# felipescoelho/w-ofdm-optimization

Hardware: AMD Instinct MI355X
Metric: OFDM symbols/sec (whole node) + BER vs reference, N=256 16-QAM (higher is better)
Workload: dtype f32

## Files before the change

include/wofdm.h:

```cpp
#ifndef WOFDM_H
#define WOFDM_H

#include <stdint.h>

#ifdef __cplusplus
extern "C" {
#endif

#define WOFDM_ABI_VERSION 1

#define WOFDM_OK            0
#define WOFDM_E_INVALID    -1
#define WOFDM_E_UNSUPPORTED -2
#define WOFDM_E_HIP        -3
#define WOFDM_E_NOMEM      -4

#define WOFDM_MAX_TAPS     21
#define WOFDM_MAX_SYMS     16

typedef struct wofdm_cfg {
    int32_t  n_fft;
    int32_t  bits_per_sc;
    int32_t  syms_per_frame;
    int32_t  cp, cs;
// ... 45 lines not shown

int wofdm_plan_dump_frame(wofdm_plan *plan, uint32_t cell, uint64_t frame,
                          const uint8_t *labels, const float *unit_noise,
                          uint64_t *counts, wofdm_dump *out);

int wofdm_plan_set_allocation(wofdm_plan *plan, const uint8_t *active);

int wofdm_plan_set_tx_mask(wofdm_plan *plan, const float *mask);

int wofdm_plan_status(wofdm_plan *plan);

int wofdm_plan_info(wofdm_plan *plan, int32_t info[5]);

int wofdm_plan_kernel_id(wofdm_plan *plan, int32_t id[2]);

int wofdm_plan_kernel_geo(wofdm_plan *plan, int32_t *id);
int wofdm_cfg_geo_id(const wofdm_cfg *cfg);

#define WOFDM_OPT_FIR_VALU       0
#define WOFDM_OPT_MAX_SPW        1
#define WOFDM_OPT_TXMASK_DIRECT  2
#define WOFDM_OPT_DFT_VALU       3
#define WOFDM_OPT_GENERIC_GEOMETRY 4
int wofdm_plan_set_option(wofdm_plan *plan, int32_t option, int32_t value);

int wofdm_run(const wofdm_cfg *cfg, int device, const float *w_tx, const float *w_rx,
              const float *h, const float *snr_db, uint64_t *counts);
int wofdm_run_injected(const wofdm_cfg *cfg, int device, const float *w_tx, const float *w_rx,
                       const float *h, const float *snr_db, const uint8_t *labels,
                       const float *unit_noise, uint64_t *counts);

int wofdm_interference(const wofdm_cfg *cfg, int device, const float *w_tx, const float *w_rx,
                       const float *h, float *power);

int wofdm_interference_masked(const wofdm_cfg *cfg, int device, const float *w_tx, const float *w_rx,
                              const float *h, const uint8_t *active ,
                              const float *tx_mask ,
                              float *power  ,
                              float *wanted );

int wofdm_tx_psd(const wofdm_cfg *cfg, int device, const float *w_tx, const float *X, int no_symbols,
                 int overlap, float *psd);

typedef struct wofdm_psd_job {
    int32_t block;
    int32_t cp, cs;
    int32_t overlap;
// ... 353 lines not shown
```

w-ofdm-optimization_amd/_lib.py:

```python
import ctypes as C
import os
import subprocess

import numpy as np

_HERE = os.path.dirname(os.path.abspath(__file__))
LIB_PATH = os.environ.get("WOFDM_LIB", os.path.join(_HERE, "libwofdm_hip.so"))
_LIB = None

WOFDM_OK = 0
ERRORS = {-1: "WOFDM_E_INVALID", -2: "WOFDM_E_UNSUPPORTED", -3: "WOFDM_E_HIP", -4: "WOFDM_E_NOMEM"}
MAX_TAPS = 21
OPTIONS = {"fir_valu": 0, "max_spw": 1, "txmask_direct": 2, "dft_valu": 3, "generic_geometry": 4}
MAX_SYMS = 16
TX_PAPR_CHUNK_BYTES = 256 << 20
TX_PAPR_MAX_PERIODS = 1 << 20
RX_PROFILE_CHUNK_BYTES = 256 << 20
SYNC_MAX_POINTS = 64
DOPPLER_MAX_TRACKS = 16
DOPPLER_MAX_KNOTS = 64
PA_LINEAR, PA_RAPP, PA_CLIP = 0, 1, 2
PA_MAX_POINTS = 16
PN_MAX_POINTS = 16
LINK_MAX_POINTS = 16
SOFT_MAX_SCALES = 16
CODE_MAX = 4
CODE_MAX_STEPS = 4608
CODE_LONG_MAX_STEPS = 1048576
LDPC_MAX_BITS = 16384

EXPORTS = (
    "wofdm_version", "wofdm_device_count", "wofdm_last_error", "wofdm_noise_len",
    "wofdm_plan_create", "wofdm_plan_destroy", "wofdm_plan_launch", "wofdm_plan_launch_timed",
    "wofdm_plan_launch_injected", "wofdm_plan_dump_frame", "wofdm_plan_info", "wofdm_run",
    "wofdm_run_injected", "wofdm_philox_kat", "wofdm_plan_set_allocation",
    "wofdm_plan_set_tx_mask", "wofdm_plan_status", "wofdm_plan_kernel_id", "wofdm_plan_set_option",
    "wofdm_interference", "wofdm_tx_psd", "wofdm_tx_psd_batch", "wofdm_tx_psd_batch_masked",
    "wofdm_interference_masked", "wofdm_tx_papr", "wofdm_tx_papr_kernel_ms",
    "wofdm_rx_profile", "wofdm_rx_profile_kernel_ms", "wofdm_plan_kernel_geo", "wofdm_cfg_geo_id",
    "wofdm_rx_profile_aci", "wofdm_rx_profile_sync", "wofdm_rx_profile_doppler",
    "wofdm_rx_profile_pa", "wofdm_tx_psd_batch_pa", "wofdm_rx_profile_pn",
    "wofdm_rx_profile_link", "wofdm_rx_profile_soft", "wofdm_rx_profile_tracking",
    "wofdm_rx_profile_coded", "wofdm_code_steps", "wofdm_viterbi_decode",
    "wofdm_viterbi_decode_long", "wofdm_rx_profile_coded_frame",
    "wofdm_ldpc_lift", "wofdm_ldpc_decode", "wofdm_rx_profile_ldpc",
)


class WofdmError(RuntimeError):
    def __init__(self, code, message):
        super().__init__("%s (%d): %s" % (ERRORS.get(code, "WOFDM_E_?"), code, message))
        self.code = code


class Cfg(C.Structure):
    _fields_ = [(n, C.c_int32) for n in (
        "n_fft", "bits_per_sc", "syms_per_frame", "cp", "cs", "tail_tx", "tail_rx", "prefix_rm",
        "circ_shift", "n_taps", "n_channels", "n_snr", "n_window_pairs",
        "noise_before_truncate")] + [
        ("frames_per_cell", C.c_uint64), ("frame_offset", C.c_uint64), ("seed", C.c_uint64)]

    @property
    def sym_len(self):
        return self.n_fft + self.cp + self.cs

    @property
    def stride(self):
        return self.sym_len - self.tail_tx
# ... 70 lines not shown
        import torch
    except ImportError:
        pass
    if not os.path.exists(LIB_PATH):
        raise ImportError(
            "%s not found: build it with `make -C %s` (hipcc, gfx950). The w-OFDM hot path has "
            "no CPU fallback." % (LIB_PATH, os.path.join(_HERE, "csrc")))
    L = C.CDLL(LIB_PATH)
    vp, u64 = C.c_void_p, C.c_uint64
    L.wofdm_version.restype = C.c_int
    L.wofdm_device_count.restype = C.c_int
    L.wofdm_last_error.restype = C.c_char_p
    L.wofdm_noise_len.argtypes = [C.POINTER(Cfg)]
    L.wofdm_plan_create.argtypes = [C.POINTER(vp), C.POINTER(Cfg), C.c_int, vp, vp, vp, vp]
    L.wofdm_plan_destroy.argtypes = [vp]
    L.wofdm_plan_launch.argtypes = [vp, u64, u64, vp, vp]
    L.wofdm_plan_launch_timed.argtypes = [vp, u64, u64, vp, vp, C.POINTER(C.c_float)]
    L.wofdm_plan_launch_injected.argtypes = [vp, u64, vp, vp, vp, vp]
    L.wofdm_plan_dump_frame.argtypes = [vp, C.c_uint32, u64, vp, vp, vp, C.POINTER(Dump)]
    L.wofdm_plan_info.argtypes = [vp, vp]
    L.wofdm_plan_kernel_id.argtypes = [vp, vp]
    L.wofdm_plan_kernel_geo.argtypes = [vp, C.POINTER(C.c_int32)]
    L.wofdm_cfg_geo_id.argtypes = [C.POINTER(Cfg)]
    L.wofdm_plan_set_allocation.argtypes = [vp, vp]
    L.wofdm_plan_set_tx_mask.argtypes = [vp, vp]
    L.wofdm_plan_status.argtypes = [vp]
    L.wofdm_plan_set_option.argtypes = [vp, C.c_int32, C.c_int32]
    L.wofdm_run.argtypes = [C.POINTER(Cfg), C.c_int, vp, vp, vp, vp, vp]
    L.wofdm_run_injected.argtypes = [C.POINTER(Cfg), C.c_int, vp, vp, vp, vp, vp, vp, vp]
    L.wofdm_philox_kat.argtypes = [C.c_int, vp, vp, vp]
    L.wofdm_interference.argtypes = [C.POINTER(Cfg), C.c_int, vp, vp, vp, vp]
    L.wofdm_interference_masked.argtypes = [C.POINTER(Cfg), C.c_int, vp, vp, vp, vp, vp, vp, vp]
    L.wofdm_tx_psd.argtypes = [C.POINTER(Cfg), C.c_int, vp, vp, C.c_int, C.c_int, vp]
    i32 = C.c_int32
    L.wofdm_tx_psd_batch.argtypes = [i32, C.c_int, i32, vp, vp, i32, i32, vp, vp]
    L.wofdm_tx_psd_batch_masked.argtypes = [i32, C.c_int, i32, vp, vp, i32, vp, vp, vp, i32, i32, vp, vp]
    L.wofdm_tx_papr.argtypes = [C.POINTER(Cfg), C.c_int, vp, vp, vp, C.c_float, C.c_float, i32, vp, vp, vp]
    L.wofdm_tx_papr_kernel_ms.argtypes = [C.POINTER(C.c_float)]
    L.wofdm_rx_profile.argtypes = [C.POINTER(Cfg), C.c_int, vp, vp, vp, vp, vp, vp, vp, vp]
    L.wofdm_rx_profile_aci.argtypes = [C.POINTER(Cfg), C.c_int, vp, vp, vp, vp, vp, vp, vp, vp, i32, C.c_float, vp, vp]
    L.wofdm_rx_profile_kernel_ms.argtypes = [C.POINTER(C.c_float)]
    L.wofdm_rx_profile_sync.argtypes = [C.POINTER(Cfg), C.c_int, vp, vp, vp, vp, vp, vp, i32, C.POINTER(SyncPoint), vp, vp, vp, vp]
    L.wofdm_rx_profile_doppler.argtypes = [C.POINTER(Cfg), C.c_int, vp, vp, vp, i32, i32, i32, vp, vp, vp, vp, vp, vp, vp]
    L.wofdm_rx_profile_pa.argtypes = [C.POINTER(Cfg), C.c_int, vp, vp, vp, vp, vp, vp, i32, C.POINTER(PaPoint), vp, vp, vp, vp, vp, vp]
    L.wofdm_rx_profile_pn.argtypes = [C.POINTER(Cfg), C.c_int, vp, vp, vp, vp, vp, vp, i32, C.POINTER(PnPoint), vp, vp, vp, vp]
    L.wofdm_rx_profile_link.argtypes = [C.POINTER(Cfg), C.c_int, vp, vp, vp, vp, vp, vp, vp, i32, i32, i32, vp, vp, vp, i32,
# ... 45 lines not shown
```

w-ofdm-optimization_amd/csrc/wofdm_abi.hip:

```cpp
#include "../../include/wofdm.h"
#include "wofdm_kernel.h"
#include "wofdm_link.h"
#include "philox.h"

#include <algorithm>
#include <cmath>
#include <complex>
#include <cstdarg>
#include <cstdio>
#include <cstdlib>
#include <cstring>
#include <mutex>
#include <utility>
#include <vector>

namespace {

thread_local char g_err[512] = "";
thread_local float g_papr_ms = 0.f;
thread_local float g_rxprof_ms = 0.f;

int fail(int code, const char *fmt, ...)
{
    va_list ap;
// ... 63 lines not shown
    geom g{};
    uint32_t n_cells = 0;
    float *d_wtx = nullptr, *d_wrx = nullptr, *d_nlin = nullptr;
    float2 *d_h = nullptr;
    int *d_geo = nullptr;
    float2 *d_nscr = nullptr;
    uint64_t nscr_elems = 0;
    wofdm_kparams base{};
    wofdm_kernel_fn fn[4] = {nullptr, nullptr, nullptr, nullptr};
    int var = WOFDM_VAR_PLAIN;
    bool has_alloc = false, has_mask = false;
    bool force_direct_mask = false;
    bool fir_valu = false;
    bool dft_valu = false;
    int max_spw = 0;
    bool generic_geo = false;
    int geo = 0;
    uint32_t *d_amask = nullptr;
    float2 *d_tmask = nullptr;
    float2 *d_tspec = nullptr;
    float *d_tspec4 = nullptr;
    unsigned *d_status = nullptr;
    unsigned long long *d_work = nullptr;
    uint32_t split_alpha_256 = WOFDM_SPLIT_ALPHA_256, split_chunk = WOFDM_SPLIT_CHUNK;
    bool split_forced = false;
    uint4 *d_fira = nullptr;
    float firm_sx = 1.f, firm_sh = 1.f;
    uint4 *d_dftc = nullptr;
    float *d_rxs = nullptr;
#ifdef WOFDM_AUDIT
    uint32_t *audit = nullptr;
    uint32_t audit_items = 0;
#endif
    int occ = 1, cus = 1, layout = 1;
    hipEvent_t ev0 = nullptr, ev1 = nullptr;
};

namespace {

size_t wofdm_amask_words(int N)
{
    const size_t NQ = (size_t)N / 4;
    return N == 256 ? 2 * NQ + 256 : NQ + (NQ > 256 ? NQ : 256);
}

int geo_id_of(const geom &g)
// ... 109 lines not shown
    fft_pow2(a, -1);
    fft_pow2(b, -1);
    for (size_t i = 0; i < Mb; ++i) a[i] *= b[i];
    fft_pow2(a, +1);
    std::vector<cplx> g((size_t)L);
    for (int n = 0; n < L; ++n) g[(size_t)n] = a[(size_t)n] * c[(size_t)n] / ((double)Mb * (double)L);
    return g;
}

void mask_fastconv_spectrum(const float *mask, int L, int MF, float2 *spec)
{
    const int P = (L + 1) / 2, G = 3 * P - 2;
    const std::vector<cplx> g = idft_any(mask, L);
    std::vector<cplx> gt((size_t)MF, cplx(0.0, 0.0));
    for (int t = 0; t < G && t < MF; ++t) gt[(size_t)t] = g[(size_t)(((t - (P - 1)) % L + L) % L)];
    fft_pow2(gt, -1);
    for (int f = 0; f < MF; ++f)
        spec[f] = make_float2((float)(gt[(size_t)f].real() / MF), (float)(gt[(size_t)f].imag() / MF));
}

std::mutex g_gate_mu;
hipEvent_t g_gate_last[64] = {};

int launch(wofdm_plan *pl, int mode, wofdm_kparams &kp, uint64_t total_items, int force_grid,
           hipStream_t stream)
{
    wofdm_kernel_fn fn = pl->fn[mode];
    if (!fn) return fail(WOFDM_E_UNSUPPORTED, "no kernel for n_fft=%d", pl->g.N);
    if (total_items == 0) return WOFDM_OK;
    uint64_t grid = (uint64_t)pl->cus * (uint64_t)pl->occ;
#ifdef WOFDM_DEV_OCC
    grid = (uint64_t)pl->cus * (uint64_t)(WOFDM_DEV_OCC);
#endif
    if (grid > total_items) grid = total_items;
    if (force_grid > 0) grid = (uint64_t)force_grid;
    const size_t row = wofdm_noise_scratch_len(pl->g.N, pl->layout);
    if (row && grid * row > pl->nscr_elems) {
        HIP_TRY(hipDeviceSynchronize());
        if (pl->d_nscr) (void)hipFree(pl->d_nscr);
        pl->d_nscr = nullptr; pl->nscr_elems = 0;
        HIP_TRY(hipMalloc(&pl->d_nscr, grid * row * sizeof(float2)));
        pl->nscr_elems = grid * row;
    }
    kp.noise_scratch = pl->d_nscr;
    kp.status = pl->d_status;
    kp.dftc = pl->d_dftc;
    kp.rx_scale = pl->d_rxs;
    const bool dynamic = (mode == WOFDM_MODE_GEN || mode == WOFDM_MODE_INJECT) && wofdm_layout_dynamic(pl->layout, pl->g.N)
                         && (pl->split_forced || (pl->occ >= 2 && total_items / grid >= WOFDM_SPLIT_MIN_ITEMS));
    const wofdm_split sp = wofdm_work_split(total_items, grid, dynamic, pl->split_alpha_256, pl->split_chunk);
    kp.head_q = sp.head_q; kp.head_r = sp.head_r; kp.tail0 = sp.tail0; kp.total = total_items;
    kp.chunk = sp.chunk;
    kp.work = pl->d_work;
    kp.lds_bytes = pl->base.lds_bytes;
    float2 *tm = pl->var == WOFDM_VAR_TXFFT ? (pl->layout == 15 ? reinterpret_cast<float2 *>(pl->d_tspec4) : pl->d_tspec) : pl->d_tmask;
    kp.tx_scale = pl->base.tx_scale;
    kp.dump_unscale_tx = pl->base.dump_unscale_tx;
    kp.dump_unscale_rx = pl->base.dump_unscale_rx;
#ifdef WOFDM_AUDIT
    kp.audit = pl->audit; kp.audit_items = pl->audit_items;
#endif
#ifdef WOFDM_DELAY
    {
        const char *dp = std::getenv("WOFDM_DELAY_POINT"), *dw = std::getenv("WOFDM_DELAY_WAVES"), *dn = std::getenv("WOFDM_DELAY_LEN");
        kp.delay_point = dp ? (uint32_t)std::strtoul(dp, nullptr, 0) : 0;
        kp.delay_waves = dw ? (uint32_t)std::strtoul(dw, nullptr, 0) : 0;
        kp.delay_len = dn ? (uint32_t)std::strtoul(dn, nullptr, 0) : 8;
    }
#endif
    void *args[] = {&kp, &pl->d_wtx, &pl->d_wrx, &pl->d_h, &pl->d_nlin, &pl->d_geo, &pl->d_amask, &tm,
                    &pl->d_fira};
    {
        std::lock_guard<std::mutex> lock(g_gate_mu);
        hipEvent_t *last = g_gate_last;
        const int dev = pl->device & 63;
        if (last[dev]) HIP_TRY(hipStreamWaitEvent(stream, last[dev], 0));
        else HIP_TRY(hipEventCreateWithFlags(&last[dev], hipEventDisableTiming));
        if (kp.tail0 < kp.total) HIP_TRY(hipMemsetAsync(pl->d_work, 0, sizeof(unsigned long long), stream));
        HIP_TRY(hipLaunchKernel(reinterpret_cast<const void *>(fn), dim3((unsigned)grid),
                                dim3(64u * (unsigned)wofdm_waves(pl->layout, pl->g.N, pl->g.S, pl->g.B)), args, kp.lds_bytes, stream));
        HIP_TRY(hipEventRecord(last[dev], stream));
    }
    return WOFDM_OK;
}

int check_status(wofdm_plan *pl)
{
    unsigned st = 0;
    HIP_TRY(hipMemcpy(&st, pl->d_status, sizeof st, hipMemcpyDeviceToHost));
    if (st != 0)
        return fail(WOFDM_E_HIP, "kernel status 0x%x: a wave timed out waiting for its workgroup "
                    "(results must not be used)", st);
    return WOFDM_OK;
}

int check_launch_args(wofdm_plan *pl, uint64_t frames_per_cell)
{
    if (!pl) return fail(WOFDM_E_INVALID, "plan is NULL");
    if (frames_per_cell > (1ull << 40)) return fail(WOFDM_E_INVALID, "frames_per_cell too large");
    return WOFDM_OK;
}
// ... 327 lines not shown
    PLAN_TRY(hipEventCreate(&pl->ev0));
    PLAN_TRY(hipEventCreate(&pl->ev1));

    int geo[WOFDM_G_COUNT];
    geo[WOFDM_G_S] = g.S; geo[WOFDM_G_MU] = g.mu; geo[WOFDM_G_RHO] = g.rho; geo[WOFDM_G_BETA] = g.beta;
    geo[WOFDM_G_DELTA] = g.delta; geo[WOFDM_G_GAMMA] = g.gamma; geo[WOFDM_G_KAPPA] = g.kappa;
    geo[WOFDM_G_L] = g.L; geo[WOFDM_G_P] = g.P; geo[WOFDM_G_B] = g.B; geo[WOFDM_G_T] = g.T;
    geo[WOFDM_G_NL] = g.NL; geo[WOFDM_G_NSNR] = cfg->n_snr; geo[WOFDM_G_NCH] = cfg->n_channels;
    geo[WOFDM_G_FBUF] = 0;
    geo[WOFDM_G_NACT] = g.N;
    geo[WOFDM_G_SPWR] = 0;
    PLAN_TRY(hipMalloc(&pl->d_geo, sizeof geo));
    PLAN_TRY(hipMemcpy(pl->d_geo, geo, sizeof geo, hipMemcpyHostToDevice));

    wofdm_kparams &kp = pl->base;
    kp.n_cells = pl->n_cells; kp.first_cell = 0; kp.inject_base_cell = 0;
    kp.seed_lo = (uint32_t)cfg->seed; kp.seed_hi = (uint32_t)(cfg->seed >> 32);

    hipDeviceProp_t prop;
    PLAN_TRY(hipGetDeviceProperties(&prop, device));
    pl->cus = prop.multiProcessorCount;
    PLAN_TRY(hipMalloc(&pl->d_status, sizeof(unsigned)));
    PLAN_TRY(hipMemset(pl->d_status, 0, sizeof(unsigned)));
    PLAN_TRY(hipMalloc(&pl->d_work, sizeof(unsigned long long)));
    PLAN_TRY(hipMemset(pl->d_work, 0, sizeof(unsigned long long)));
    if (const char *e = std::getenv("WOFDM_SPLIT_ALPHA")) {
        const double a = std::strtod(e, nullptr);
        if (!(a >= 0.0 && a < 1.0)) {
            wofdm_plan_destroy(pl);
            return fail(WOFDM_E_INVALID, "WOFDM_SPLIT_ALPHA=%s: a fraction in [0, 1)", e);
        }
        pl->split_alpha_256 = (uint32_t)(a * 256.0);
        pl->split_forced = true;
    }
    if (const char *e = std::getenv("WOFDM_SPLIT_CHUNK")) {
        const unsigned long c = std::strtoul(e, nullptr, 0);
        if (c < 1 || c > (1ul << 20)) {
            wofdm_plan_destroy(pl);
            return fail(WOFDM_E_INVALID, "WOFDM_SPLIT_CHUNK=%s: 1 ... 2^20 items", e);
        }
        pl->split_chunk = (uint32_t)c;
        pl->split_forced = true;
    }
    if ((rc = configure(pl)) != WOFDM_OK) {
        wofdm_plan_destroy(pl);
        return rc;
    }
    const int occ = pl->occ;
    if (const size_t row = wofdm_noise_scratch_len(g.N, pl->layout)) {
        pl->nscr_elems = (uint64_t)pl->cus * (uint64_t)occ * row;
        PLAN_TRY(hipMalloc(&pl->d_nscr, pl->nscr_elems * sizeof(float2)));
        PLAN_TRY(hipMemset(pl->d_nscr, 0, pl->nscr_elems * sizeof(float2)));
        PLAN_TRY(hipDeviceSynchronize());
    }
#undef PLAN_TRY
    *out = pl;
    return WOFDM_OK;
}

int wofdm_plan_destroy(wofdm_plan *pl)
{
    if (!pl) return WOFDM_OK;
    (void)hipSetDevice(pl->device);
    if (pl->d_wtx) (void)hipFree(pl->d_wtx);
    if (pl->d_wrx) (void)hipFree(pl->d_wrx);
    if (pl->d_h) (void)hipFree(pl->d_h);
    if (pl->d_nlin) (void)hipFree(pl->d_nlin);
    if (pl->d_geo) (void)hipFree(pl->d_geo);
    if (pl->d_nscr) (void)hipFree(pl->d_nscr);
    if (pl->d_amask) (void)hipFree(pl->d_amask);
    if (pl->d_tmask) (void)hipFree(pl->d_tmask);
// ... 126 lines not shown
    pl->has_mask = true;
    const int rc = configure(pl);
    if (rc != WOFDM_OK) pl->has_mask = had;
    return rc;
}

int wofdm_plan_set_option(wofdm_plan *pl, int32_t option, int32_t value)
{
    if (!pl) return fail(WOFDM_E_INVALID, "plan is NULL");
    HIP_TRY(hipSetDevice(pl->device));
    HIP_TRY(hipDeviceSynchronize());
    const bool direct = pl->force_direct_mask, valu = pl->fir_valu, dvalu = pl->dft_valu, ggeo = pl->generic_geo;
    const int cap = pl->max_spw;
    switch (option) {
    case WOFDM_OPT_FIR_VALU: pl->fir_valu = value != 0; break;
    case WOFDM_OPT_MAX_SPW:
        if (value != 0 && value != 1 && value != 2 && value != 4)
            return fail(WOFDM_E_INVALID, "WOFDM_OPT_MAX_SPW takes 0, 1, 2 or 4");
        pl->max_spw = value;
        break;
    case WOFDM_OPT_TXMASK_DIRECT: pl->force_direct_mask = value != 0; break;
    case WOFDM_OPT_DFT_VALU: pl->dft_valu = value != 0; break;
    case WOFDM_OPT_GENERIC_GEOMETRY: pl->generic_geo = value != 0; break;
    default: return fail(WOFDM_E_INVALID, "unknown option %d", (int)option);
    }
    const int rc = configure(pl);
    if (rc != WOFDM_OK) { pl->force_direct_mask = direct; pl->fir_valu = valu; pl->max_spw = cap; pl->dft_valu = dvalu; pl->generic_geo = ggeo; }
    if (rc == WOFDM_OK) {
        const size_t row = wofdm_noise_scratch_len(pl->g.N, pl->layout);
        const uint64_t wgs = (uint64_t)pl->cus * (uint64_t)pl->occ;
        if (row && wgs * row > pl->nscr_elems) {
            if (pl->d_nscr) (void)hipFree(pl->d_nscr);
            pl->d_nscr = nullptr; pl->nscr_elems = 0;
            HIP_TRY(hipMalloc(&pl->d_nscr, wgs * row * sizeof(float2)));
            HIP_TRY(hipMemset(pl->d_nscr, 0, wgs * row * sizeof(float2)));
            pl->nscr_elems = wgs * row;
        }
    }
    return rc;
}

int wofdm_plan_status(wofdm_plan *pl)
{
    if (!pl) return fail(WOFDM_E_INVALID, "plan is NULL");
    HIP_TRY(hipSetDevice(pl->device));
    return check_status(pl);
// ... 10 lines not shown
    return WOFDM_OK;
}

#ifdef WOFDM_AUDIT
extern "C" int wofdm_plan_set_audit(wofdm_plan *pl, void *dev, uint32_t items)
{
    if (!pl) return WOFDM_E_INVALID;
    pl->audit = static_cast<uint32_t *>(dev); pl->audit_items = items;
    return WOFDM_OK;
}
#endif
int wofdm_plan_kernel_id(wofdm_plan *pl, int32_t id[2])
{
    if (!pl || !id) return fail(WOFDM_E_INVALID, "NULL argument");
    id[0] = pl->layout;
    id[1] = pl->var;
    return WOFDM_OK;
}

int wofdm_plan_kernel_geo(wofdm_plan *pl, int32_t *id)
{
    if (!pl || !id) return fail(WOFDM_E_INVALID, "NULL argument");
    *id = pl->geo;
    return WOFDM_OK;
}

int wofdm_cfg_geo_id(const wofdm_cfg *cfg)
{
    geom g;
    const int rc = check_cfg(cfg, &g);
    return rc != WOFDM_OK ? rc : geo_id_of(g);
}

int wofdm_plan_launch(wofdm_plan *pl, uint64_t frame_offset, uint64_t frames_per_cell,
                      uint64_t *counts_dev, void *stream)
{
    int rc = check_launch_args(pl, frames_per_cell);
    if (rc) return rc;
    if (!counts_dev) return fail(WOFDM_E_INVALID, "counts_dev is NULL");
    HIP_TRY(hipSetDevice(pl->device));
    wofdm_kparams kp = pl->base;
    kp.frames_per_cell = frames_per_cell; kp.frame_offset = frame_offset;
    kp.counts = reinterpret_cast<unsigned long long *>(counts_dev);
    return launch(pl, WOFDM_MODE_GEN, kp, frames_per_cell * pl->n_cells, 0,
                  static_cast<hipStream_t>(stream));
}
// ... 1734 lines not shown
```

w-ofdm-optimization_amd/csrc/wofdm_kernel.h:

```cpp
#pragma once
#include <hip/hip_runtime.h>
#include <stdint.h>

#define WOFDM_LT 21

struct wofdm_kdump {
    uint8_t *labels_tx;
    float2  *X, *tx, *conv, *rx, *Y, *Xhat;
    uint8_t *labels_rx;
    float   *gain;
    float2  *unit_noise;
    float2  *sink;
};

template <int N, bool NOTW = false> struct wofdm_lds {
    static constexpr int TAIL_MAX = 16, CPCS_MAX = N >= 1024 ? 64 : 128, TAILRX_MAX = 64;
    static constexpr int off_tw = 0;
    static constexpr int TW_BYTES = NOTW ? 0 : (N == 256 || N == 512 ? 6 * 64 * 16 : 8 * N);
    static constexpr int off_g = off_tw + TW_BYTES;
    static constexpr int off_sums = off_g + 8 * N;
    static constexpr int off_flags = off_sums + 4 * 64;
    static constexpr int off_wtx = off_flags + 4 * 64;
    static constexpr int off_wrx = off_wtx + 4 * (N + CPCS_MAX);
    static constexpr int off_lut = off_wrx + 4 * (N + TAILRX_MAX);
    static constexpr int off_fbuf = off_lut + 8 * 64;
};

enum { WOFDM_G_S, WOFDM_G_MU, WOFDM_G_RHO, WOFDM_G_BETA, WOFDM_G_DELTA, WOFDM_G_GAMMA, WOFDM_G_KAPPA,
       WOFDM_G_L, WOFDM_G_P, WOFDM_G_B, WOFDM_G_T, WOFDM_G_NL, WOFDM_G_NSNR, WOFDM_G_NCH, WOFDM_G_FBUF,
       WOFDM_G_NACT,
       WOFDM_G_SPWR,
       WOFDM_G_COUNT };

struct wofdm_kparams {
    uint32_t n_cells;
    uint32_t first_cell;
    uint32_t inject_base_cell;
    unsigned lds_bytes;
    uint64_t frames_per_cell, frame_offset;
    uint64_t head_q, head_r, tail0, total;
    uint32_t chunk;
    unsigned long long *work;
    uint32_t seed_lo, seed_hi;
    unsigned long long *counts;
    const uint4 *dftc;
    const float *rx_scale;
    const uint8_t *labels;
    const float2  *unit_noise;
    float2 *noise_scratch;
    unsigned *status;
    float tx_scale, dump_unscale_tx, dump_unscale_rx;
    wofdm_kdump dump;
#ifdef WOFDM_DELAY
    uint32_t delay_point, delay_waves, delay_len;
#endif
#ifdef WOFDM_AUDIT
    uint32_t *audit;
    uint32_t audit_items;
#endif
};

static constexpr bool wofdm_layout_dynamic(int layout, int n_fft)
{
    return layout == 10 || layout == 11 || layout == 13 || layout == 14 || layout == 16 || (layout == 12 && n_fft == 512);
}
#define WOFDM_SPLIT_ALPHA_256 192
#define WOFDM_SPLIT_CHUNK 8
#define WOFDM_SPLIT_MIN_ITEMS 512
struct wofdm_split { uint64_t head_q, head_r, tail0; uint32_t chunk; };
static inline wofdm_split wofdm_work_split(uint64_t total, uint64_t grid, bool dynamic, uint32_t alpha_256, uint32_t chunk)
{
    const uint64_t q = total / grid;
    if (!dynamic || total <= grid) return {q, total % grid, total, 0u};
    const uint64_t head = (q >> 8) * alpha_256 + (((q & 255u) * alpha_256) >> 8);
    return {head, 0u, head * grid, chunk};
}

#ifndef WOFDM_NOISE_SCRATCH_MIN_N
#define WOFDM_NOISE_SCRATCH_MIN_N 1024
#endif
static inline int wofdm_cpcs_max(int n_fft) { return n_fft >= 1024 ? 64 : 128; }
static inline int wofdm_kslot(int k) { return k == 6 ? 8 : k; }
static constexpr int wofdm_fir8_tiles(int n_fft) { return n_fft >= 1024 ? 9 : (n_fft >= 512 ? 5 : 3); }
// ... 356 lines not shown
```

w-ofdm-optimization_amd/csrc/wofdm_kernel.hip:

```cpp
#include "wofdm_kernel.h"
#include "wofdm_device.h"
#include "philox.h"
#include <type_traits>
#include <utility>

#ifndef WOFDM_FAULT_SKIP_FLAG
#define WOFDM_FAULT_SKIP_FLAG 0
#endif
#define WOFDM_UNIT_BUILD (WOFDM_FAULT_SKIP_FLAG ? 1 : 0)


#define PRIO_LATENCY 2
#define PRIO_TRANSFORM 1
#define PRIO_TILES 0
#define WAVE_PRIO(x) __builtin_amdgcn_s_setprio(x)

namespace {

#ifdef WOFDM_STAMP
#define STAMP(slot)                                                                            \
    do {                                                                                       \
        __builtin_amdgcn_sched_barrier(0);                                                     \
        const unsigned long long now_ = __builtin_amdgcn_s_memtime();                          \
        __builtin_amdgcn_s_waitcnt(0xC07F);                                                    \
// ... 477 lines not shown
    constexpr bool FIR8M = LI.masked;
    constexpr bool FIRQ = LI.fir == WOFDM_FIR_QUARTER, FIR8 = LI.fir == WOFDM_FIR_ONE, FIRM = FIRQ || FIR8;
    constexpr int SPW = LI.spw;
    constexpr int NT = LI.nt, PRE = WOFDM_FIRM_PRE;
    constexpr int VT = WOFDM_FIR8_VT;
    constexpr bool ALLOC = VAR >= 1, TXMASK = VAR == 2, TXFFT = VAR == 3;
    constexpr bool RELAX = !DUMP && VAR < 2;
    constexpr bool RELAXM = !DUMP && VAR >= 2;
    constexpr bool RELAXF = RELAX || RELAXM;
    static_assert(!(TXMASK || TXFFT) || SPW == 1, "the Tx mask stage runs one symbol per wave");
    constexpr int LT = WOFDM_LT;
    constexpr int BPL = geo<N>::BPL, NQ = geo<N>::NQ;
    constexpr bool FULL = geo<N>::FULL;
    constexpr bool QW = SPW == 4 && !MDFT && !MDS;
    constexpr int VS = QW ? 1 : (MDS ? 1 : SPW), VB = QW ? 4 : BPL;
    constexpr int RB = fir_geo<N, LAY>::RB, NBK = fir_geo<N, LAY>::NBK;
    constexpr bool EVEN = fir_geo<N, LAY>::EVEN;
    constexpr bool RENOISE = N >= WOFDM_NOISE_SCRATCH_MIN_N;
    constexpr bool RELAUNDER = N >= 1024 || (N >= 512 && VAR >= 2);
    constexpr int LW_MIN = FIR8 ? N : 0;
    extern __shared__ __attribute__((aligned(16))) unsigned char smem[];

    const int tid = threadIdx.x, lane0 = tid & 63;
    const int wv = __builtin_amdgcn_readfirstlane(tid >> 6);
    const int SPWR = PART ? __builtin_amdgcn_readfirstlane(gm[WOFDM_G_SPWR]) : SPW, SPWR2 = SPWR >> 1;
    (void)SPWR2;
    const int s0 = wv * SPWR;
    int lane = lane0;
#define GEO_PHASE()                                                                            \
    int goff_ = 0;                     \
    if constexpr (GEO == 0) asm volatile("" : "+s"(goff_));    \
    const auto gq = gm + goff_

    using L = wofdm_lds<N, MDS>;
    v2f *tw = reinterpret_cast<v2f *>(smem + L::off_tw);
    v2f *G = reinterpret_cast<v2f *>(smem + L::off_g);
    float *sums = reinterpret_cast<float *>(smem + L::off_sums);
    lds_vint *flags = (lds_vint *)(smem + L::off_flags);
    float *wtx = reinterpret_cast<float *>(smem + L::off_wtx);
    float *wrx = reinterpret_cast<float *>(smem + L::off_wrx);
    v2f *qlut = reinterpret_cast<v2f *>(smem + L::off_lut);
    v2f *fbuf = reinterpret_cast<v2f *>(smem + L::off_fbuf);
    const v2f *g_h = reinterpret_cast<const v2f *>(g_h_);
    uint32_t *Hp = reinterpret_cast<uint32_t *>(smem + L::off_fbuf);
#define TAILS()                                                                                \
    const int tail_off = gq[WOFDM_G_FBUF];                            \
    v2f *tailb = fbuf + tail_off;                                                                 \
    uint32_t *tH = reinterpret_cast<uint32_t *>(tailb), *tL = tH + gq[WOFDM_G_S] * gq[WOFDM_G_BETA]; \
    (void)tH; (void)tL; (void)tail_off

    DELAY_AT(11);
    for (int i = tid; i < gm[WOFDM_G_FBUF]; i += blockDim.x) fbuf[i] = mk(0.f, 0.f);
    if (tid < 64) flags[tid] = 0;
    enum { WS_OFF_LO = 17, WS_OFF_HI = 18,
           WS_CHUNK = 19,
           WS_LEFT_LO = 21, WS_LEFT_HI = 22,
           WS_TAIL0_LO = 23, WS_TAIL0_HI = 28,
           WS_WORK_LO = 29, WS_WORK_HI = 30,
           WS_CELL0 = 31 };
    constexpr bool DYN = !DUMP && wofdm_layout_dynamic(LAY, N);
    if (DYN && tid == 0) {
        const uint64_t left = p.total - p.tail0, wp = (uint64_t)(uintptr_t)p.work;
        flags[WS_CHUNK] = (int)p.chunk;
        flags[WS_LEFT_LO] = (int)(uint32_t)left; flags[WS_LEFT_HI] = (int)(uint32_t)(left >> 32);
        flags[WS_TAIL0_LO] = (int)(uint32_t)p.tail0; flags[WS_TAIL0_HI] = (int)(uint32_t)(p.tail0 >> 32);
        flags[WS_WORK_LO] = (int)(uint32_t)wp; flags[WS_WORK_HI] = (int)(uint32_t)(wp >> 32);
        flags[WS_CELL0] = (int)p.first_cell;
    }
    if (tid < 64) sums[tid] = 0.f;
    int iter = 0;
    if constexpr (MDS) {
    } else if constexpr (MPIPE) {
        u4 *dl = reinterpret_cast<u4 *>(smem + L::off_tw);
        const u4 *dg = reinterpret_cast<const u4 *>(p.dftc);
        for (int i = tid; i < 6 * 64; i += blockDim.x) dl[i] = dg[i < 256 ? i : i + 256];
    } else if constexpr (QW) fill_twiddles_qw(tw, tid, (int)blockDim.x);
    else fill_twiddles<N>(tw, tid, (int)blockDim.x);
    if (tid < (1 << K)) {
        constexpr int hb = K >> 1, mm = (1 << hb) - 1;
        constexpr float qs = K == 2 ? 0.70710678118654752f : (K == 4 ? 0.31622776601683794f
                                                                     : 0.15430334996209191f);
        const uint32_t gi = (uint32_t)tid >> hb, gq = (uint32_t)tid & (uint32_t)mm;
// ... 3 lines not shown
            reinterpret_cast<uint32_t *>(qlut)[tid] = __builtin_bit_cast(uint32_t, w);
        } else {
            qlut[tid] = mk((float)(2 * li - mm), (float)(mm - 2 * lq)) * qs;
        }
    }
    constexpr float qscale = K == 2 ? 0.70710678118654752f : (K == 4 ? 0.31622776601683794f : 0.15430334996209191f);
    const uint32_t *qlw = reinterpret_cast<const uint32_t *>(qlut);
    (void)qlw;
    v2f *rg = fbuf + gm[WOFDM_G_FBUF] + gm[WOFDM_G_S] * gm[WOFDM_G_BETA];
    if constexpr (TXMASK) {
        const int Lm = 2 * gm[WOFDM_G_P] - 1;
        for (int t = tid; t < mask_geo<N>::RG_LEN; t += blockDim.x) {
            int kk = (t - mask_geo<N>::RG_OFF) % Lm;
            if (kk < 0) kk += Lm;
            rg[t] = ldg2(g_tmask + kk);
        }
    }
    v2f *mtw = fbuf + gm[WOFDM_G_FBUF] + gm[WOFDM_G_S] * gm[WOFDM_G_BETA];
    v2f *mscr = mtw + maskfft_geo::MF;
    if constexpr (TXFFT && !MDM) fill_twiddles<maskfft_geo::MF>(mtw, tid, (int)blockDim.x);
    constexpr int MDM_PK = 344;
    v2f *mdm_park = reinterpret_cast<v2f *>(smem + ((L::off_fbuf + 8 * (gm[WOFDM_G_FBUF] + gm[WOFDM_G_S] * gm[WOFDM_G_BETA]) + 15) & ~15));
    (void)mdm_park;
    __syncthreads();
    DELAY_AT(12);

    constexpr int k = K, half = K >> 1, m1 = (1 << half) - 1;
    constexpr uint32_t lmask = (1u << K) - 1u;
    constexpr float qinv = K == 2 ? 1.4142135623730951f : (K == 4 ? 3.1622776601683795f
                                                                   : 6.4807406984078604f);
    constexpr int ks = K == 6 ? 8 : K;
    constexpr int bps = N * ks / 128;
    static_assert(SPW * bps <= 64, "data-bit blocks of a wave must fit one pass");

    const uint64_t F = p.frames_per_cell;
    const int n_ch = gm[WOFDM_G_NCH], n_snr = gm[WOFDM_G_NSNR];
    uint64_t n_items = p.head_q + (blockIdx.x < p.head_r ? 1u : 0u), fidx = 0;
    uint32_t cell = 0;
    int ch = 0, sn = 0, pair = 0;
    auto ws_get = [&](int i) { return __builtin_amdgcn_readfirstlane((uint32_t)flags[i]); };
    auto ws_get64 = [&](int lo, int hi) { return ((uint64_t)ws_get(hi) << 32) | ws_get(lo); };
    auto seek = [&](uint64_t item, uint32_t first_cell) {
        uint32_t f_lo = (uint32_t)F, f_hi = (uint32_t)(F >> 32);
        uint32_t nc = (uint32_t)n_ch, ns = (uint32_t)n_snr;
        if constexpr (DYN) asm volatile("" : "+s"(f_lo), "+s"(f_hi), "+s"(nc), "+s"(ns));
        const uint64_t Fd = ((uint64_t)f_hi << 32) | f_lo;
        const uint32_t cell_rel = (uint32_t)(item / Fd);
// ... 2261 lines not shown
                    a[0] = ab; a[1] = as; a[2] = __float_as_uint(aud_g); a[3] = __float_as_uint(aud_ps);
                    a[4] = __float_as_uint(aud_pn); a[5] = __builtin_amdgcn_s_getreg(4 | (31 << 11));
                    a[6] = __builtin_amdgcn_s_getreg(20 | (31 << 11)); a[7] = (uint32_t)__builtin_amdgcn_s_memtime();
                }
            }
#endif
        }
        STAMP(6);
        if (++fidx == F) { fidx = 0; next_cell(); }
    }
#ifdef WOFDM_STAMP
    STAMP(7);
#endif
    if constexpr (DYN) {
        const uint32_t chunk = ws_get(WS_CHUNK);
        if (chunk == 0 || !take_chunk(chunk)) break;
    } else break;
    }
    if (cur_cell != 0xFFFFFFFFu) flush(cur_cell);
    if constexpr (RELAXF) {
        __syncthreads();
        if (tid == 0 && flags[20] != 0) atomicOr(p.status, 1u);
    }
#ifdef WOFDM_STAMP
    if (lane0 == 0) {
        unsigned long long *dst = p.counts + 4 * (size_t)(p.first_cell + p.n_cells)
                                  + ((size_t)blockIdx.x * 16 + wv) * 16;
        for (int i = 0; i < 16; ++i) dst[i] = stamp_acc[i];
    }
#endif
}

template <int N, int K, int LAY, int VAR> wofdm_kernel_fn pick_mode(int mode)
{
    if constexpr (wofdm_layout_built(LAY, N, VAR)) {
        switch (mode) {
        case WOFDM_MODE_GEN: return wofdm_frames_kernel<N, K, LAY, false, false, VAR>;
        case WOFDM_MODE_INJECT: return wofdm_frames_kernel<N, K, LAY, true, false, VAR>;
        case WOFDM_MODE_DUMP_GEN: return wofdm_frames_kernel<N, K, LAY, false, true, VAR>;
        case WOFDM_MODE_DUMP_INJECT: return wofdm_frames_kernel<N, K, LAY, true, true, VAR>;
        }
    }
    return nullptr;
}

template <int N, int K, int LAY> wofdm_kernel_fn pick_var(int mode, int var)
// ... 56 lines not shown
```

w-ofdm-optimization_amd/simulation.py:

```python
import ctypes as C
import os

import numpy as np

from . import _lib
from . import variants as V


def _diag_or_vec(w, n):
    w = np.asarray(w)
    if w.ndim == 2 and w.shape[0] == w.shape[1]:
        w = np.diag(w)
    w = np.asarray(w, dtype=np.float64).reshape(-1)
    if w.size != n:
        raise ValueError("window has %d samples, expected %d" % (w.size, n))
    return w


def make_cfg(st, bits_per_sc, syms_per_frame, n_taps, n_channels, n_snr, n_window_pairs,
             noise_before_truncate=True, seed=0, frames_per_cell=0, frame_offset=0):
    return _lib.Cfg(st.n_fft, bits_per_sc, syms_per_frame, st.cp, st.cs, st.tail_tx, st.tail_rx,
                    st.prefix_rm, st.circ_shift, n_taps, n_channels, n_snr, n_window_pairs,
                    1 if noise_before_truncate else 0, frames_per_cell, frame_offset, seed)

# ... 32 lines not shown
        except Exception:
            pass

    @property
    def counts_shape(self):
        c = self.cfg
        return (c.n_window_pairs, c.n_snr, c.n_channels, 4)

    def info(self):
        a = (C.c_int32 * 5)()
        _lib.check(self.lib.wofdm_plan_info(self._h_plan, a))
        return dict(waves_per_workgroup=a[0], lds_bytes=a[1], workgroups=a[2],
                    workgroups_per_cu=a[3], compute_units=a[4])

    def kernel_id(self):
        a = (C.c_int32 * 2)()
        _lib.check(self.lib.wofdm_plan_kernel_id(self._h_plan, a))
        return int(a[0]), int(a[1])

    def kernel_geo(self):
        a = C.c_int32()
        _lib.check(self.lib.wofdm_plan_kernel_geo(self._h_plan, C.byref(a)))
        return int(a.value)

    def set_allocation(self, active):
        if active is None:
            _lib.check(self.lib.wofdm_plan_set_allocation(self._h_plan, None))
            self.n_active = self.cfg.n_fft
            return
        a = np.ascontiguousarray(np.asarray(active).reshape(-1) != 0, dtype=np.uint8)
        if a.shape != (self.cfg.n_fft,):
            raise ValueError("allocation must have n_fft = %d entries" % self.cfg.n_fft)
        _lib.check(self.lib.wofdm_plan_set_allocation(self._h_plan, a.ctypes.data))
        self.n_active = int(a.sum())

    def set_tx_mask(self, mask):
        if mask is None:
            _lib.check(self.lib.wofdm_plan_set_tx_mask(self._h_plan, None))
            return
        m = _lib.f32(np.asarray(mask).reshape(-1), (2 * self.cfg.sym_len - 1,))
        _lib.check(self.lib.wofdm_plan_set_tx_mask(self._h_plan, m.ctypes.data))

    def set_option(self, name, value):
        _lib.check(self.lib.wofdm_plan_set_option(self._h_plan, _lib.OPTIONS[name], int(value)))

    def new_counts(self):
# ... 230 lines not shown
```

Baseline: 1.238 billion.

## Add optional SIMD-aware wave role rotation with per-CU ticket census

Adds an option that rotates the logical wave index inside each workgroup. The rotation is chosen from the hardware SIMD id and a per-CU atomic ticket, so that co-resident workgroups on a CU put different roles on different SIMDs. The aim is to balance work across SIMDs when wave roles are uneven. It is off by default. On the GEO>0 generation path, each launch still pays for a hw_id read, one global atomic per workgroup, a census record write, and a larger work buffer. A host API is added to read back the census.

```diff
diff --git a/include/wofdm.h b/include/wofdm.h
--- a/include/wofdm.h
+++ b/include/wofdm.h
@@ -91,7 +91,12 @@
 #define WOFDM_OPT_TXMASK_DIRECT  2
 #define WOFDM_OPT_DFT_VALU       3
 #define WOFDM_OPT_GENERIC_GEOMETRY 4
+#define WOFDM_OPT_WAVE_ROLES     5
+#define WOFDM_WAVE_ROLES_DEFAULT 0
 int wofdm_plan_set_option(wofdm_plan *plan, int32_t option, int32_t value);
+
+int wofdm_plan_wave_roles(wofdm_plan *plan, int32_t *records, int32_t capacity, int32_t *n_records);
+int wofdm_wave_role_base(const int32_t simd[4], uint32_t ticket);
 
 int wofdm_run(const wofdm_cfg *cfg, int device, const float *w_tx, const float *w_rx,
               const float *h, const float *snr_db, uint64_t *counts);
diff --git a/w-ofdm-optimization_amd/_lib.py b/w-ofdm-optimization_amd/_lib.py
--- a/w-ofdm-optimization_amd/_lib.py
+++ b/w-ofdm-optimization_amd/_lib.py
@@ -11,7 +11,7 @@
 WOFDM_OK = 0
 ERRORS = {-1: "WOFDM_E_INVALID", -2: "WOFDM_E_UNSUPPORTED", -3: "WOFDM_E_HIP", -4: "WOFDM_E_NOMEM"}
 MAX_TAPS = 21
-OPTIONS = {"fir_valu": 0, "max_spw": 1, "txmask_direct": 2, "dft_valu": 3, "generic_geometry": 4}
+OPTIONS = {"fir_valu": 0, "max_spw": 1, "txmask_direct": 2, "dft_valu": 3, "generic_geometry": 4, "wave_roles": 5}
 MAX_SYMS = 16
 TX_PAPR_CHUNK_BYTES = 256 << 20
 TX_PAPR_MAX_PERIODS = 1 << 20
@@ -44,6 +44,7 @@
     "wofdm_rx_profile_coded", "wofdm_code_steps", "wofdm_viterbi_decode",
     "wofdm_viterbi_decode_long", "wofdm_rx_profile_coded_frame",
     "wofdm_ldpc_lift", "wofdm_ldpc_decode", "wofdm_rx_profile_ldpc",
+    "wofdm_plan_wave_roles", "wofdm_wave_role_base",
 )
 
 
@@ -160,6 +161,8 @@
     L.wofdm_plan_kernel_id.argtypes = [vp, vp]
     L.wofdm_plan_kernel_geo.argtypes = [vp, C.POINTER(C.c_int32)]
     L.wofdm_cfg_geo_id.argtypes = [C.POINTER(Cfg)]
+    L.wofdm_plan_wave_roles.argtypes = [vp, vp, C.c_int32, C.POINTER(C.c_int32)]
+    L.wofdm_wave_role_base.argtypes = [C.POINTER(C.c_int32), C.c_uint32]
     L.wofdm_plan_set_allocation.argtypes = [vp, vp]
     L.wofdm_plan_set_tx_mask.argtypes = [vp, vp]
     L.wofdm_plan_status.argtypes = [vp]
diff --git a/w-ofdm-optimization_amd/csrc/wofdm_abi.hip b/w-ofdm-optimization_amd/csrc/wofdm_abi.hip
--- a/w-ofdm-optimization_amd/csrc/wofdm_abi.hip
+++ b/w-ofdm-optimization_amd/csrc/wofdm_abi.hip
@@ -109,6 +109,10 @@
     float *d_tspec4 = nullptr;
     unsigned *d_status = nullptr;
     unsigned long long *d_work = nullptr;
+    uint64_t role_records = 0;
+    bool wave_roles = WOFDM_WAVE_ROLES_DEFAULT != 0;
+    uint64_t last_grid = 0;
+    bool last_roles = false, last_spread = false;
     uint32_t split_alpha_256 = WOFDM_SPLIT_ALPHA_256, split_chunk = WOFDM_SPLIT_CHUNK;
     bool split_forced = false;
     uint4 *d_fira = nullptr;
@@ -264,6 +268,16 @@
 std::mutex g_gate_mu;
 hipEvent_t g_gate_last[64] = {};
 
+int alloc_work(wofdm_plan *pl, uint64_t records)
+{
+    if (pl->d_work) (void)hipFree(pl->d_work);
+    pl->d_work = nullptr; pl->role_records = 0;
+    HIP_TRY(hipMalloc(&pl->d_work, wofdm_role_bytes(records)));
+    HIP_TRY(hipMemset(pl->d_work, 0, wofdm_role_bytes(records)));
+    pl->role_records = records;
+    return WOFDM_OK;
+}
+
 int launch(wofdm_plan *pl, int mode, wofdm_kparams &kp, uint64_t total_items, int force_grid,
            hipStream_t stream)
 {
@@ -284,6 +298,13 @@
         HIP_TRY(hipMalloc(&pl->d_nscr, grid * row * sizeof(float2)));
         pl->nscr_elems = grid * row;
     }
+    const bool roles = mode == WOFDM_MODE_GEN && pl->geo > 0;
+    if (roles && grid > pl->role_records) {
+        HIP_TRY(hipDeviceSynchronize());
+        const int rc = alloc_work(pl, grid);
+        if (rc != WOFDM_OK) return rc;
+    }
+    kp.role_spread = pl->wave_roles ? 1u : 0u;
     kp.noise_scratch = pl->d_nscr;
     kp.status = pl->d_status;
     kp.dftc = pl->d_dftc;
@@ -318,7 +339,10 @@
         const int dev = pl->device & 63;
         if (last[dev]) HIP_TRY(hipStreamWaitEvent(stream, last[dev], 0));
         else HIP_TRY(hipEventCreateWithFlags(&last[dev], hipEventDisableTiming));
-        if (kp.tail0 < kp.total) HIP_TRY(hipMemsetAsync(pl->d_work, 0, sizeof(unsigned long long), stream));
+        const bool spread = roles && pl->wave_roles;
+        if (spread) HIP_TRY(hipMemsetAsync(pl->d_work, 0, wofdm_role_bytes(grid), stream));
+        else if (kp.tail0 < kp.total) HIP_TRY(hipMemsetAsync(pl->d_work, 0, sizeof(unsigned long long), stream));
+        pl->last_grid = grid; pl->last_roles = roles; pl->last_spread = spread;
         HIP_TRY(hipLaunchKernel(reinterpret_cast<const void *>(fn), dim3((unsigned)grid),
                                 dim3(64u * (unsigned)wofdm_waves(pl->layout, pl->g.N, pl->g.S, pl->g.B)), args, kp.lds_bytes, stream));
         HIP_TRY(hipEventRecord(last[dev], stream));
@@ -692,8 +716,8 @@
     pl->cus = prop.multiProcessorCount;
     PLAN_TRY(hipMalloc(&pl->d_status, sizeof(unsigned)));
     PLAN_TRY(hipMemset(pl->d_status, 0, sizeof(unsigned)));
-    PLAN_TRY(hipMalloc(&pl->d_work, sizeof(unsigned long long)));
-    PLAN_TRY(hipMemset(pl->d_work, 0, sizeof(unsigned long long)));
+    PLAN_TRY(hipMalloc(&pl->d_work, wofdm_role_bytes(0)));
+    PLAN_TRY(hipMemset(pl->d_work, 0, wofdm_role_bytes(0)));
     if (const char *e = std::getenv("WOFDM_SPLIT_ALPHA")) {
         const double a = std::strtod(e, nullptr);
         if (!(a >= 0.0 && a < 1.0)) {
@@ -717,6 +741,10 @@
         return rc;
     }
     const int occ = pl->occ;
+    if (alloc_work(pl, (uint64_t)pl->cus * (uint64_t)occ) != WOFDM_OK) {
+        wofdm_plan_destroy(pl);
+        return WOFDM_E_HIP;
+    }
     if (const size_t row = wofdm_noise_scratch_len(g.N, pl->layout)) {
         pl->nscr_elems = (uint64_t)pl->cus * (uint64_t)occ * row;
         PLAN_TRY(hipMalloc(&pl->d_nscr, pl->nscr_elems * sizeof(float2)));
@@ -889,6 +917,7 @@
     case WOFDM_OPT_TXMASK_DIRECT: pl->force_direct_mask = value != 0; break;
     case WOFDM_OPT_DFT_VALU: pl->dft_valu = value != 0; break;
     case WOFDM_OPT_GENERIC_GEOMETRY: pl->generic_geo = value != 0; break;
+    case WOFDM_OPT_WAVE_ROLES: pl->wave_roles = value != 0; break;
     default: return fail(WOFDM_E_INVALID, "unknown option %d", (int)option);
     }
     const int rc = configure(pl);
@@ -945,6 +974,40 @@
 {
     if (!pl || !id) return fail(WOFDM_E_INVALID, "NULL argument");
     *id = pl->geo;
+    return WOFDM_OK;
+}
+
+int wofdm_wave_role_base(const int32_t simd[4], uint32_t ticket)
+{
+    if (!simd) return fail(WOFDM_E_INVALID, "NULL argument");
+    return wofdm_role_base(simd[0], simd[1], simd[2], simd[3], ticket);
+}
+
+int wofdm_plan_wave_roles(wofdm_plan *pl, int32_t *records, int32_t capacity, int32_t *n_records)
+{
+    if (!pl || !n_records || capacity < 0 || (capacity > 0 && !records)) return fail(WOFDM_E_INVALID, "NULL argument or negative capacity");
+    HIP_TRY(hipSetDevice(pl->device));
+    HIP_TRY(hipDeviceSynchronize());
+    const uint64_t grid = pl->last_grid;
+    *n_records = (int32_t)std::min<uint64_t>(grid, 0x7fffffffu);
+    const size_t n = (size_t)std::min<uint64_t>(grid, (uint64_t)capacity);
+    if (!pl->last_roles) {
+        for (size_t i = 0; i < n; ++i) {
+            int32_t *r = records + 8 * i;
+            r[0] = -1; r[1] = 0; r[2] = r[3] = r[4] = r[5] = -1; r[6] = 0; r[7] = 0;
+        }
+        return WOFDM_OK;
+    }
+    std::vector<uint32_t> raw(n * WOFDM_ROLE_WORDS);
+    if (n) HIP_TRY(hipMemcpy(raw.data(), wofdm_role_census(pl->d_work), raw.size() * sizeof(uint32_t), hipMemcpyDeviceToHost));
+    for (size_t i = 0; i < n; ++i) {
+        const uint32_t *w = raw.data() + i * WOFDM_ROLE_WORDS;
+        int32_t *r = records + 8 * i;
+        if (!(w[WOFDM_ROLE_BASE] & 0x100u)) return fail(WOFDM_E_HIP, "workgroup %zu of the last launch left no census record", i);
+        r[0] = (int32_t)w[WOFDM_ROLE_KEY]; r[1] = pl->last_spread ? (int32_t)w[WOFDM_ROLE_TICKET] : -1;
+        for (int j = 0; j < 4; ++j) r[2 + j] = (int32_t)((w[WOFDM_ROLE_SIMDS] >> (8 * j)) & 255u);
+        r[6] = (int32_t)(w[WOFDM_ROLE_BASE] & 3u); r[7] = 1;
+    }
     return WOFDM_OK;
 }
 
diff --git a/w-ofdm-optimization_amd/csrc/wofdm_kernel.h b/w-ofdm-optimization_amd/csrc/wofdm_kernel.h
--- a/w-ofdm-optimization_amd/csrc/wofdm_kernel.h
+++ b/w-ofdm-optimization_amd/csrc/wofdm_kernel.h
@@ -40,6 +40,7 @@
     uint64_t frames_per_cell, frame_offset;
     uint64_t head_q, head_r, tail0, total;
     uint32_t chunk;
+    uint32_t role_spread;
     unsigned long long *work;
     uint32_t seed_lo, seed_hi;
     unsigned long long *counts;
@@ -59,6 +60,31 @@
     uint32_t audit_items;
 #endif
 };
+static_assert(sizeof(wofdm_kparams) % 8 == 0 && offsetof(wofdm_kparams, work) == 72 && offsetof(wofdm_kparams, dump) == 160, "wofdm_kparams moved");
+
+__host__ __device__ constexpr int wofdm_role_base(int s0, int s1, int s2, int s3, uint32_t ticket)
+{
+    if (((1u << (s0 & 31)) | (1u << (s1 & 31)) | (1u << (s2 & 31)) | (1u << (s3 & 31))) != 15u) return 0;
+    const int t = (int)(ticket & 3u);
+    return s0 == t ? 0 : (s1 == t ? 1 : (s2 == t ? 2 : 3));
+}
+#define WOFDM_ROLE_KEYS 4096
+__host__ __device__ constexpr uint32_t wofdm_role_cu_key(uint32_t hw_id, uint32_t xcc_id)
+{
+    return ((xcc_id & 15u) << 8) | ((hw_id >> 8) & 255u);
+}
+__host__ __device__ constexpr uint32_t wofdm_role_simd(uint32_t hw_id) { return (hw_id >> 4) & 3u; }
+enum { WOFDM_ROLE_KEY, WOFDM_ROLE_TICKET, WOFDM_ROLE_SIMDS, WOFDM_ROLE_BASE, WOFDM_ROLE_WORDS };
+#define WOFDM_ROLE_HEAD 64
+__host__ __device__ inline uint32_t *wofdm_role_tickets(unsigned long long *work)
+{
+    return reinterpret_cast<uint32_t *>(work) + WOFDM_ROLE_HEAD / sizeof(uint32_t);
+}
+__host__ __device__ inline uint32_t *wofdm_role_census(unsigned long long *work) { return wofdm_role_tickets(work) + WOFDM_ROLE_KEYS; }
+static inline size_t wofdm_role_bytes(uint64_t workgroups)
+{
+    return WOFDM_ROLE_HEAD + sizeof(uint32_t) * (WOFDM_ROLE_KEYS + (size_t)workgroups * WOFDM_ROLE_WORDS);
+}
 
 static constexpr bool wofdm_layout_dynamic(int layout, int n_fft)
 {
diff --git a/w-ofdm-optimization_amd/csrc/wofdm_kernel.hip b/w-ofdm-optimization_amd/csrc/wofdm_kernel.hip
--- a/w-ofdm-optimization_amd/csrc/wofdm_kernel.hip
+++ b/w-ofdm-optimization_amd/csrc/wofdm_kernel.hip
@@ -523,10 +523,9 @@
     extern __shared__ __attribute__((aligned(16))) unsigned char smem[];
 
     const int tid = threadIdx.x, lane0 = tid & 63;
-    const int wv = __builtin_amdgcn_readfirstlane(tid >> 6);
+    int wv = __builtin_amdgcn_readfirstlane(tid >> 6);
     const int SPWR = PART ? __builtin_amdgcn_readfirstlane(gm[WOFDM_G_SPWR]) : SPW, SPWR2 = SPWR >> 1;
     (void)SPWR2;
-    const int s0 = wv * SPWR;
     int lane = lane0;
 #define GEO_PHASE()                                                                            \
     int goff_ = 0;                     \
@@ -558,7 +557,8 @@
            WS_LEFT_LO = 21, WS_LEFT_HI = 22,
            WS_TAIL0_LO = 23, WS_TAIL0_HI = 28,
            WS_WORK_LO = 29, WS_WORK_HI = 30,
-           WS_CELL0 = 31 };
+           WS_CELL0 = 31,
+           WS_ROLE = 8 };
     constexpr bool DYN = !DUMP && wofdm_layout_dynamic(LAY, N);
     if (DYN && tid == 0) {
         const uint64_t left = p.total - p.tail0, wp = (uint64_t)(uintptr_t)p.work;
@@ -608,7 +608,31 @@
     constexpr int MDM_PK = 344;
     v2f *mdm_park = reinterpret_cast<v2f *>(smem + ((L::off_fbuf + 8 * (gm[WOFDM_G_FBUF] + gm[WOFDM_G_S] * gm[WOFDM_G_BETA]) + 15) & ~15));
     (void)mdm_park;
+    if constexpr (GEO > 0) {
+        static_assert(GEO == 0 || wofdm_waves(LAY, N, wofdm_geo_row_of(GEO).S, wofdm_geo_row_of(GEO).B) == 4, "wave roles: four waves");
+        uint32_t *role_w = reinterpret_cast<uint32_t *>(smem + L::off_g);
+        const uint32_t hw_id = __builtin_amdgcn_s_getreg(4 | (31 << 11));
+        if (lane0 == 0) role_w[tid >> 6] = wofdm_role_simd(hw_id);
+        if (tid == 0) {
+            const uint32_t key = wofdm_role_cu_key(hw_id, __builtin_amdgcn_s_getreg(20 | (31 << 11)));
+            role_w[4] = key;
+            role_w[5] = __hip_atomic_fetch_add(wofdm_role_tickets(p.work) + key, 1u, __ATOMIC_RELAXED, __HIP_MEMORY_SCOPE_AGENT);
+        }
+    }
     __syncthreads();
+    if constexpr (GEO > 0) {
+        const uint32_t *role_w = reinterpret_cast<const uint32_t *>(smem + L::off_g);
+        const uint32_t r0 = role_w[0], r1 = role_w[1], r2 = role_w[2], r3 = role_w[3], ticket = role_w[5];
+        const int base = p.role_spread ? wofdm_role_base((int)r0, (int)r1, (int)r2, (int)r3, ticket) : 0;
+        if (tid == 0) {
+            flags[WS_ROLE + WOFDM_ROLE_KEY] = (int)role_w[4];
+            flags[WS_ROLE + WOFDM_ROLE_TICKET] = (int)ticket;
+            flags[WS_ROLE + WOFDM_ROLE_SIMDS] = (int)(r0 | (r1 << 8) | (r2 << 16) | (r3 << 24));
+            flags[WS_ROLE + WOFDM_ROLE_BASE] = (int)(0x100u | (uint32_t)base);
+        }
+        wv = __builtin_amdgcn_readfirstlane(((tid >> 6) - base) & 3);
+    }
+    const int s0 = wv * SPWR;
     DELAY_AT(12);
 
     constexpr int k = K, half = K >> 1, m1 = (1 << half) - 1;
@@ -2916,6 +2940,15 @@
         __syncthreads();
         if (tid == 0 && flags[20] != 0) atomicOr(p.status, 1u);
     }
+    if constexpr (GEO > 0) {
+        static_assert(GEO == 0 || DYN, "wave roles: the work counter's address is in the LDS words of the hand-out");
+        if (tid == 0) {
+            typedef __attribute__((address_space(1))) uint32_t gu32;
+            gu32 *rec = (gu32 *)(((uint64_t)(uint32_t)flags[WS_WORK_HI] << 32) | (uint32_t)flags[WS_WORK_LO])
+                        + (WOFDM_ROLE_HEAD / sizeof(uint32_t) + WOFDM_ROLE_KEYS) + (size_t)blockIdx.x * WOFDM_ROLE_WORDS;
+            for (int i = 0; i < WOFDM_ROLE_WORDS; ++i) rec[i] = (uint32_t)flags[WS_ROLE + i];
+        }
+    }
 #ifdef WOFDM_STAMP
     if (lane0 == 0) {
         unsigned long long *dst = p.counts + 4 * (size_t)(p.first_cell + p.n_cells)
diff --git a/w-ofdm-optimization_amd/simulation.py b/w-ofdm-optimization_amd/simulation.py
--- a/w-ofdm-optimization_amd/simulation.py
+++ b/w-ofdm-optimization_amd/simulation.py
@@ -78,6 +78,13 @@
         a = C.c_int32()
         _lib.check(self.lib.wofdm_plan_kernel_geo(self._h_plan, C.byref(a)))
         return int(a.value)
+
+    def wave_roles(self):
+        n = C.c_int32()
+        _lib.check(self.lib.wofdm_plan_wave_roles(self._h_plan, None, 0, C.byref(n)))
+        rec = np.zeros((n.value, 8), np.int32)
+        _lib.check(self.lib.wofdm_plan_wave_roles(self._h_plan, rec.ctypes.data, n.value, C.byref(n)))
+        return rec[:n.value]
 
     def set_allocation(self, active):
         if active is None:
```

After: 1.238 billion, median of 6. No clear change (+0.0%).
